# ZooMEISTER/vickers-hardness-Unet

Measured on AMD Instinct MI355X. Metric: 512x512 images/sec (train fwd+bwd), higher is better.
Workload: dtype bf16

## Files before the change

### vickers-hardness-unet_amd/csrc/conv_bwd_onepass.hip

```cpp
#include <stdlib.h>

#include <string>
#include <type_traits>

#include "vk_common.h"

namespace vk {

void launch_slab_reduce(size_t n4, int splits, const float* slab, float* dw, hipStream_t st);

struct OnePassParams {
  const void *g, *z, *z1, *w;
  void* y;
  const float *coef, *scale, *shift, *bnr_scale, *bnr_shift;
  double* sums;
  float* slab;
  int N, H, W, RS, RSsum, relu;
  uint32_t w_bytes, t_bytes;
};

template <int CK>
struct OnePassCfg {
  static constexpr int NSTEP = CK == 16 ? 5 : 9;
  static constexpr int APS = CK == 16 ? 48 : 96;
  static constexpr int VPP = CK / 8;
  static constexpr int NVEC = 18 * VPP;
  static constexpr int NLD = (NVEC + 63) / 64;
  static constexpr int ROWB = CK == 16 ? 1024 : 2048;
  static constexpr int V_OFF = 4 * ROWB, ZERO_OFF = 8 * ROWB;
  static constexpr int WAVE_LDS = 8 * ROWB + 64;
  static constexpr int RED = CK * 9 * CK * 4;
  static constexpr int SMEM = 4 * WAVE_LDS > RED ? 4 * WAVE_LDS : RED;
  static_assert(18 * APS <= ROWB && NLD <= 2, "row image");
};

template <typename T, int CK>
__global__ __launch_bounds__(256, (CK == 16 ? 2 : 1)) void conv_bwd_onepass_kernel(const OnePassParams p) {
  using Cfg = OnePassCfg<CK>;
  constexpr int NSTEP = Cfg::NSTEP, APS = Cfg::APS, VPP = Cfg::VPP, NVEC = Cfg::NVEC, NLD = Cfg::NLD, ROWB = Cfg::ROWB;
  constexpr int VE = 8, TC = CK / 16;
  static_assert(sizeof(T) == 2, "16-bit element types");
  extern __shared__ __attribute__((aligned(16))) char smem[];
  typedef __attribute__((address_space(3))) s16x4_t* lds_s16x4_ptr;
  const int RS = p.RS;
  const int tid = threadIdx.x, lane = tid & 63;
  const int wave = __builtin_amdgcn_readfirstlane(tid >> 6);
  char* const ring = smem + wave * Cfg::WAVE_LDS;
  char* const vring = ring + Cfg::V_OFF;
  const int strips_x = (p.W + 15) / 16, strips_y = (p.H + RS - 1) / RS;
  int sid = (int)blockIdx.x * 4 + wave;
  const bool active = sid < p.N * strips_y * strips_x;
  const int strip = sid;
  const int sx = sid % strips_x;
  sid /= strips_x;
  const int sy = sid % strips_y;
  const int n = sid / strips_y;
  const int x0 = sx * 16, ys = sy * RS, ye = min(p.H, ys + RS);
  const int li = lane & 15, kg = lane >> 4;

  f32x4_t wacc[9][TC][TC];
#pragma unroll
  for (int t = 0; t < 9; ++t)
#pragma unroll
    for (int a = 0; a < TC; ++a)
#pragma unroll
      for (int b = 0; b < TC; ++b) wacc[t][a][b] = f32x4_t{0.f, 0.f, 0.f, 0.f};

  if (active) {
    const __amdgpu_buffer_rsrc_t rsg = make_rsrc(p.g, p.t_bytes);
    const __amdgpu_buffer_rsrc_t rsz = make_rsrc(p.z, p.t_bytes);
    const __amdgpu_buffer_rsrc_t rs1 = make_rsrc(p.z1, p.t_bytes);
    const __amdgpu_buffer_rsrc_t rsw = make_rsrc(p.w, p.w_bytes);

    u32x4_t wf[NSTEP][TC];
#pragma unroll
    for (int st = 0; st < NSTEP; ++st)
#pragma unroll
      for (int a = 0; a < TC; ++a) {
        const int row = a * 16 + li;
        uint32_t off;
        bool ok = true;
        if (CK == 16) {
          const int tap = 2 * st + (kg >> 1);
          ok = tap < 9;
          off = (uint32_t)(((row * 9 + (8 - tap)) * 16 + (kg & 1) * VE) * 2);
        } else {
          const int pos = kg ^ (((row >> 2) & 1) << 1);
          off = (uint32_t)((((8 - st) * CK + row) * 4 + pos) * 16);
        }
        wf[st][a] = buf_load16(rsw, ok ? off : kOOB);
      }
    if (lane < 4) *reinterpret_cast<u32x4_t*>(ring + Cfg::ZERO_OFF + lane * 16) = u32x4_t{0, 0, 0, 0};

    int st_off[NLD], ld_col[NLD];
    bool xok[NLD];
#pragma unroll
    for (int q = 0; q < NLD; ++q) {
      const int v = lane + 64 * q;
      int hx = v / VPP, hv = v % VPP;
      if (VPP == 4) {
        if ((hx | 3) < 18) hx = (hx & ~3) | ((hx & 1) << 1) | ((hx >> 1) & 1);
      } else {
        if ((v | 15) < NVEC) { hx = (v & 7) | ((v >> 4) << 3); hv = (v >> 3) & 1; }
      }
      const int xs = x0 - 1 + hx;
      xok[q] = v < NVEC && (unsigned)xs < (unsigned)p.W;
      ld_col[q] = xs * CK + hv * VE;
      st_off[q] = v < NVEC ? hx * APS + hv * 16 : -1;
    }
    static_assert(VPP == 4 || NLD == 1, "C = 16: one staged vector per lane");
    const int hvl = VPP == 4 ? lane % VPP : (((lane | 15) < NVEC) ? (lane >> 3) & 1 : lane % VPP);
    const bool aff = p.scale != nullptr, relu = p.relu != 0;
    float sc[VE], sh[VE], ca[VE], cb[VE], cc[VE];
#pragma unroll
    for (int j = 0; j < VE; ++j) {
      sc[j] = aff ? p.scale[hvl * VE + j] : 1.f;
      sh[j] = aff ? p.shift[hvl * VE + j] : 0.f;
      ca[j] = p.coef[hvl * VE + j];
      cb[j] = p.coef[CK + hvl * VE + j];
      cc[j] = p.coef[2 * CK + hvl * VE + j];
    }
    struct RowQ {
      u32x4_t g[NLD], z[NLD], v[NLD];
    };
    auto issue = [&](int j, RowQ& r) {
      const bool rok = (unsigned)j < (unsigned)p.H;
#pragma unroll
      for (int q = 0; q < NLD; ++q) {
        const uint32_t off = (rok && xok[q]) ? (uint32_t)(((n * p.H + j) * p.W) * CK + ld_col[q]) * 2u : kOOB;
        r.g[q] = buf_load16(rsg, off);
        r.z[q] = buf_load16(rsz, off);
        r.v[q] = buf_load16(rs1, off);
      }
    };
    auto write_row = [&](int j, const RowQ& r) {
      const bool rok = (unsigned)j < (unsigned)p.H;
      const int slot = (j & 3) * ROWB;
#pragma unroll
      for (int q = 0; q < NLD; ++q) {
        if (st_off[q] < 0) continue;
        float gf[VE], zf[VE], o[VE];
        Vec16<T>::unpack(r.g[q], gf);
        Vec16<T>::unpack(r.z[q], zf);
#pragma unroll
        for (int e = 0; e < VE; ++e) o[e] = fmaf(ca[e], gf[e], fmaf(cb[e], zf[e], cc[e]));
        u32x4_t dz = Vec16<T>::pack(o);
        u32x4_t v = r.v[q];
        if (aff) v = AffineRelu<T>::run(v, sc, sh, relu);
        if (!(rok && xok[q])) {
          dz = u32x4_t{0, 0, 0, 0};
          v = u32x4_t{0, 0, 0, 0};
        }
        *reinterpret_cast<u32x4_t*>(ring + slot + st_off[q]) = dz;
        *reinterpret_cast<u32x4_t*>(vring + slot + st_off[q]) = v;
      }
    };

    int fr_r16[CK == 16 ? NSTEP : 1], fr_off16[CK == 16 ? NSTEP : 1];
    if (CK == 16) {
#pragma unroll
      for (int st = 0; st < NSTEP; ++st) {
        const int tap = 2 * st + (kg >> 1);
        const int r = tap / 3, sxx = tap - r * 3;
        fr_r16[st] = tap < 9 ? r : -100;
        fr_off16[st] = (li + sxx) * APS + (kg & 1) * 16;
      }
    }
    const int fr_base32 = kg * 16;
    const int lane_t = (4 * kg + (li >> 2)) * APS + (4 * (lane & 3)) * 2;
    auto tr = [](const char* q) { return __builtin_bit_cast(u32x2_t, __builtin_amdgcn_ds_read_tr16_b64_v4i16((lds_s16x4_ptr)(q))); };

// ... 50 lines not shown
    write_row(ys, pre[0]);
    auto row = [&](int y, auto ph_c) {
      constexpr int PH = decltype(ph_c)::value;
      write_row(y + 1, pre[(PH + 1) & 3]);
      issue(y + 4, pre[PH & 3]);
      z_issue(y + 1, zq[(PH & 1) ^ 1]);
      f32x4_t acc[TC];
#pragma unroll
      for (int a = 0; a < TC; ++a) acc[a] = f32x4_t{0.f, 0.f, 0.f, 0.f};
#pragma unroll
      for (int st = 0; st < NSTEP; ++st) {
        int addr;
        if (CK == 16) {
          const int vrow = y - 1 + fr_r16[st];
          addr = fr_r16[st] < 0 ? Cfg::ZERO_OFF : (vrow & 3) * ROWB + fr_off16[st];
        } else {
          const int r = st / 3, sxx = st - r * 3;
          addr = ((y - 1 + r) & 3) * ROWB + (li + sxx) * APS + fr_base32;
        }
        const u32x4_t xf = *reinterpret_cast<const u32x4_t*>(ring + addr);
#pragma unroll
        for (int a = 0; a < TC; ++a) acc[a] = Mma<T>::run(wf[st][a], xf, acc[a]);
      }
      __builtin_amdgcn_sched_barrier(0);
      const bool y_ok = y < p.H;
#pragma unroll
      for (int a = 0; a < TC; ++a) {
        float f[4] = {acc[a][0], acc[a][1], acc[a][2], acc[a][3]};
        (void)round_t(f);
        finish(a, f, y_ok ? out_off(a, y) : kOOB, x_ok && y_ok, zq[PH & 1][a]);
      }
      if constexpr ((PH & 1) == 1) {
        constexpr int SL = (PH + 3) & 3, SH = PH & 3;
        u32x4_t zf[TC];
#pragma unroll
        for (int a = 0; a < TC; ++a) {
          const u32x2_t lo = tr(ring + SL * ROWB + APS + lane_t + a * 32), hi = tr(ring + SH * ROWB + APS + lane_t + a * 32);
          zf[a] = u32x4_t{lo[0], lo[1], hi[0], hi[1]};
        }
#pragma unroll
        for (int r = 0; r < 3; ++r) {
          const int slo = ((PH + 2 + r) & 3) * ROWB, shi = ((PH + 3 + r) & 3) * ROWB;
#pragma unroll
          for (int s_ = 0; s_ < 3; ++s_) {
            u32x4_t vf[TC];
#pragma unroll
            for (int b = 0; b < TC; ++b) {
              const u32x2_t lo = tr(vring + slo + s_ * APS + lane_t + b * 32), hi = tr(vring + shi + s_ * APS + lane_t + b * 32);
              vf[b] = u32x4_t{lo[0], lo[1], hi[0], hi[1]};
            }
#pragma unroll
            for (int a = 0; a < TC; ++a)
#pragma unroll
              for (int b = 0; b < TC; ++b) wacc[r * 3 + s_][a][b] = Mma<T>::run(zf[a], vf[b], wacc[r * 3 + s_][a][b]);
          }
        }
      }
    };
    double* const sp = p.sums + (size_t)(strip % VK_STATS_REPLICAS) * 2 * CK;
    auto flush_sums = [&]() {
#pragma unroll
      for (int a = 0; a < TC; ++a)
#pragma unroll
        for (int e = 0; e < 4; ++e) {
          const float u = row16_sum(s1[a][e]), v = row16_sum(s2[a][e]);
          const int ch = a * 16 + kg * 4 + e;
          if (li == 0) {
            atomicAdd(sp + ch, (double)u);
            atomicAdd(sp + CK + ch, (double)v);
          }
          s1[a][e] = 0.f; s2[a][e] = 0.f;
        }
    };
    const int RSsum = p.RSsum;
    for (int yb = ys, left = RSsum; yb < ye; yb += 4) {
      row(yb, std::integral_constant<int, 0>{});
      row(yb + 1, std::integral_constant<int, 1>{});
      row(yb + 2, std::integral_constant<int, 2>{});
      row(yb + 3, std::integral_constant<int, 3>{});
      left -= 4;
      if (left == 0 || yb + 4 >= ye) {
        flush_sums();
        left = RSsum;
      }
    }
  }

  __syncthreads();
  float* const red = reinterpret_cast<float*>(smem);
#pragma unroll 1
  for (int phase = 0; phase < 4; ++phase) {
    if (wave == phase) {
#pragma unroll
      for (int t = 0; t < 9; ++t)
#pragma unroll
        for (int a = 0; a < TC; ++a)
#pragma unroll
          for (int b = 0; b < TC; ++b)
#pragma unroll
            for (int e = 0; e < 4; ++e) {
              const int k = a * 16 + kg * 4 + e, c = b * 16 + li;
              float* dst = red + (k * 9 + t) * CK + c;
              if (phase > 0) *dst += wacc[t][a][b][e];
              else *dst = wacc[t][a][b][e];
            }
    }
    __syncthreads();
  }
  float* const slab = p.slab + (size_t)blockIdx.x * CK * 9 * CK;
  for (int i = tid; i < CK * 9 * CK / 4; i += 256) *reinterpret_cast<f32x4_t*>(slab + i * 4) = *reinterpret_cast<const f32x4_t*>(red + i * 4);
}

template <typename T, int CK>
static int launch_onepass(OnePassParams p, float* dw, size_t slab_bytes, hipStream_t st) {
  using Cfg = OnePassCfg<CK>;
  const char* e_rs = getenv("VK_STREAM_RS");
  int RS = 256;
  if (e_rs) {
    RS = atoi(e_rs);
  } else {
    const long per_row_block = (long)p.N * ((p.W + 15) / 16), resident = CK == 16 ? 2048 : 1024;
    while (RS > 32 && per_row_block * ((p.H + RS - 1) / RS) < resident) RS >>= 1;
  }
  RS = (RS + 7) & ~7;
  if (RS < 8) RS = 8;
  int RSsum = RS;
  if (!e_rs) {
    const long per_row_block = (long)p.N * ((p.W + 15) / 16);
    RSsum = 32;
    while (RSsum * 2 <= 256 && per_row_block * ((p.H + 2 * RSsum - 1) / (2 * RSsum)) >= 4096) RSsum *= 2;
    if (RS < RSsum) RS = RSsum;
  }
  p.RSsum = RSsum;
  p.RS = RS;
  const long strips = (long)p.N * ((p.H + RS - 1) / RS) * ((p.W + 15) / 16);
  const long nwg = (strips + 3) / 4;
  if ((size_t)nwg * CK * 9 * CK * sizeof(float) > slab_bytes) return VK_ERR_UNSUPPORTED;
  static bool attr_done = false;
  if (!attr_done && Cfg::SMEM > 64 * 1024) {
    VK_CHECK_HIP(hipFuncSetAttribute((const void*)conv_bwd_onepass_kernel<T, CK>, hipFuncAttributeMaxDynamicSharedMemorySize, Cfg::SMEM));
    attr_done = true;
  }
  {
    static const std::string tag = std::string("bwd_onepass_16b_c") + std::to_string(CK);
    const double px = (double)p.N * p.H * p.W;
    vkh::ProfScope ps(tag.c_str(), st, 2.0 * 2.0 * px * CK * 9.0 * CK, 4.0 * px * CK * 2.0 + 9.0 * CK * CK * (2.0 + 4.0));
    hipLaunchKernelGGL((conv_bwd_onepass_kernel<T, CK>), dim3((unsigned)nwg), dim3(256), Cfg::SMEM, st, p);
  }
  launch_slab_reduce((size_t)CK * 9 * CK / 4, (int)nwg, p.slab, dw, st);
  VK_CHECK_HIP(hipGetLastError());
  return VK_OK;
}

}

extern "C" int vk_conv_bwd_onepass(const vk_conv_desc* d, const void* g, const void* z, const float* coef_abc, const void* w_dgrad, void* y,
                                   const vk_bnr* bnr, float* dw, void* workspace, size_t workspace_bytes, void* stream) {
  VK_CHECK_ARG(d && g && z && coef_abc && w_dgrad && y && bnr && dw, "vk_conv_bwd_onepass: null argument");
  if (d->dtype != VK_BF16 && d->dtype != VK_F16) return VK_ERR_UNSUPPORTED;
  if (d->R != 3 || d->S != 3 || d->stride != 1 || d->pad != 1 || d->transposed || d->H != d->Ho || d->W != d->Wo) return VK_ERR_UNSUPPORTED;
  if (d->src1.ptr || d->src0.up || d->src0.C != d->K || (d->K != 16 && d->K != 32)) return VK_ERR_UNSUPPORTED;
  if ((size_t)d->N * d->H * d->W * d->K * 2 >= (1ull << 31)) return VK_ERR_UNSUPPORTED;
  if (!workspace || (reinterpret_cast<uintptr_t>(workspace) & 15)) return VK_ERR_UNSUPPORTED;
  VK_CHECK_ARG(d->src0.ptr && d->N > 0 && d->H > 0 && d->W > 0, "vk_conv_bwd_onepass: empty descriptor");
  VK_CHECK_ARG((d->src0.scale != nullptr) == (d->src0.shift != nullptr), "vk_conv_bwd_onepass: scale and shift come together");
  VK_CHECK_ARG(bnr->z == d->src0.ptr && !bnr->mask && !bnr->accumulate && bnr->sums && bnr->scale && bnr->shift,
               "vk_conv_bwd_onepass: bnr must describe the layer's own input (z = src0.ptr, scale, shift, sums; no mask, no accumulate)");
  vk::OnePassParams p;
  p.g = g; p.z = z; p.z1 = d->src0.ptr; p.w = w_dgrad; p.y = y;
  p.coef = coef_abc; p.scale = d->src0.scale; p.shift = d->src0.shift; p.relu = d->src0.relu;
  p.bnr_scale = bnr->scale; p.bnr_shift = bnr->shift; p.sums = bnr->sums;
  p.slab = (float*)workspace;
  p.N = d->N; p.H = d->H; p.W = d->W; p.RS = 0;
  p.w_bytes = (uint32_t)((size_t)d->K * 9 * d->K * 2);
  p.t_bytes = (uint32_t)((size_t)d->N * d->H * d->W * d->K * 2);
  hipStream_t st = (hipStream_t)stream;
  if (d->dtype == VK_BF16)
    return d->K == 16 ? vk::launch_onepass<vk::bf16_t, 16>(p, dw, workspace_bytes, st) : vk::launch_onepass<vk::bf16_t, 32>(p, dw, workspace_bytes, st);
  return d->K == 16 ? vk::launch_onepass<vk::f16_t, 16>(p, dw, workspace_bytes, st) : vk::launch_onepass<vk::f16_t, 32>(p, dw, workspace_bytes, st);
}
```

### vickers-hardness-unet_amd/csrc/engine.hip

```cpp
#include <stdarg.h>
#include <stdio.h>
#include <stdlib.h>
#include <string.h>

#include <algorithm>
#include <atomic>
#include <map>
#include <mutex>
#include <string>
#include <vector>

#include "vk_common.h"

namespace vkh {
static thread_local char g_err[512] = "";
void set_error(const char* fmt, ...) {
  va_list ap;
  va_start(ap, fmt);
  vsnprintf(g_err, sizeof(g_err), fmt, ap);
  va_end(ap);
}

struct ProfRec {
  std::string tag;
// ... 1164 lines not shown
    xd = bn_act(h, c2);
  }
  vk_src hs = to_src(xd);
  if (h->classes == 1) RET_IF(vk_head_fwd(dt, N, S, SW, &hs, h->params + h->head_w_off, h->params + h->head_b_off, logits, st));
  else RET_IF(vk_head_fwd_multi(dt, N, S, SW, h->classes, &hs, h->params + h->head_w_off, h->params + h->head_b_off, logits, st));
  if (training) {
    if (h->bn_frozen_fwd) hipLaunchKernelGGL(k_inc_i64_masked, dim3(1), dim3(64), 0, st, (int)h->bns.size(), h->nbt, h->bn_frozen_fwd);
    else hipLaunchKernelGGL(k_inc_i64, dim3(1), dim3(64), 0, st, (int)h->bns.size(), h->nbt);
    VK_CHECK_HIP(hipGetLastError());
  }
  return VK_OK;
}

extern "C" int vk_unet_loss_ex(vk_unet* h, int mode, const void* logits, const void* target, float* loss_out, float grad_scale,
                               float w_ce, float w_dice, void* stream) {
  VK_CHECK_ARG(h && h->bound && logits && target && loss_out, "vk_unet_loss_ex: plan not bound or null tensor");
  VK_CHECK_ARG(mode == VK_LOSS_BINARY || mode == VK_LOSS_MULTILABEL || mode == VK_LOSS_MULTICLASS, "vk_unet_loss_ex: bad mode %d", mode);
  VK_CHECK_ARG(mode != VK_LOSS_BINARY || h->classes == 1, "vk_unet_loss_ex: the binary loss needs classes == 1 (the plan has %d)", h->classes);
  VK_CHECK_ARG(mode != VK_LOSS_MULTICLASS || h->classes >= 2, "vk_unet_loss_ex: the multi-class loss needs classes >= 2");
  if (h->classes == 1) return vk_unet_loss(h, (const float*)logits, (const float*)target, loss_out, grad_scale, w_ce, w_dice, stream);
  const int N = h->cfg.N, HW = h->cfg.size * h->cfg.width;
  float* dl = h->cfg.training ? (float*)(h->ws + h->off_dlogits) : nullptr;
  if (mode == VK_LOSS_MULTILABEL)
    return vk_multilabel_loss(N, h->classes, HW, (const float*)logits, (const float*)target, h->ws + h->off_mloss, h->mloss_bytes, loss_out,
                              dl, grad_scale, w_ce, w_dice, stream);
  return vk_multiclass_loss(N, h->classes, HW, (const float*)logits, (const int64_t*)target, h->ws + h->off_mloss, h->mloss_bytes, loss_out,
                            dl, grad_scale, w_ce, w_dice, stream);
}

extern "C" int vk_unet_loss_cfg(vk_unet* h, const vk_seg_loss_cfg* cfg, const void* logits, const void* target, float* loss_out,
                                float grad_scale, void* stream) {
  VK_CHECK_ARG(h && h->bound && cfg && logits && target && loss_out, "vk_unet_loss_cfg: plan not bound or null argument");
  float* dl = h->cfg.training ? (float*)(h->ws + h->off_dlogits) : nullptr;
  return vk_seg_loss(cfg, h->cfg.N, h->classes, h->cfg.size * h->cfg.width, (const float*)logits, target, h->ws + h->off_sloss,
                     h->sloss_bytes, loss_out, dl, grad_scale, stream);
}

extern "C" int vk_unet_loss_lovasz(vk_unet* h, const vk_seg_loss_cfg* seg_cfg, const vk_lovasz_cfg* lovasz_cfg, float w_lovasz,
                                   const void* logits, const void* target, void* workspace, size_t workspace_bytes, float* loss_out,
                                   float grad_scale, void* stream) {
  VK_CHECK_ARG(h && h->bound && lovasz_cfg && logits && target && workspace && loss_out,
               "vk_unet_loss_lovasz: plan not bound or null argument");
  VK_CHECK_ARG(w_lovasz == w_lovasz && w_lovasz - w_lovasz == 0.f, "vk_unet_loss_lovasz: w_lovasz is not finite");
  VK_CHECK_ARG(!seg_cfg || seg_cfg->mode == lovasz_cfg->mode, "vk_unet_loss_lovasz: the two parts disagree on the mode");
  const int N = h->cfg.N, HW = h->cfg.size * h->cfg.width;
  float* dl = h->cfg.training ? (float*)(h->ws + h->off_dlogits) : nullptr;
  hipStream_t st = (hipStream_t)stream;
  if (seg_cfg) RET_IF(vk_seg_loss(seg_cfg, N, h->classes, HW, (const float*)logits, target, h->ws + h->off_sloss, h->sloss_bytes, loss_out,
                                  dl, grad_scale, stream));
  else VK_CHECK_HIP(hipMemsetAsync(loss_out, 0, 8 * sizeof(float), st));
  RET_IF(vk_lovasz_loss(lovasz_cfg, N, h->classes, HW, (const float*)logits, target, workspace, workspace_bytes, loss_out + 8, dl,
                        grad_scale * w_lovasz, seg_cfg ? 1 : 0, stream));
  return vk::lovasz_combine(loss_out, w_lovasz, st);
}

extern "C" int vk_unet_loss(vk_unet* h, const float* logits, const float* target, float* loss_out, float grad_scale, float w_bce,
                            float w_dice, void* stream) {
  VK_CHECK_ARG(h && h->bound && logits && target && loss_out, "vk_unet_loss: plan not bound or null tensor");
  VK_CHECK_ARG(h->classes == 1, "vk_unet_loss: the binary loss needs classes == 1; use vk_unet_loss_ex");
  const size_t count = (size_t)h->cfg.N * h->cfg.size * h->cfg.width;
  float* dl = h->cfg.training ? (float*)(h->ws + h->off_dlogits) : nullptr;
  return vk_bce_dice_loss(count, logits, target, (double*)(h->ws + h->off_loss_sums), loss_out, dl, grad_scale, w_bce, w_dice, stream);
}

#ifndef VK_BN_APPLY_FUSED_MAXC_DEFAULT
#define VK_BN_APPLY_FUSED_MAXC_DEFAULT 0
#endif
namespace {

int bn_bwd_phase2(vk_unet* h, BnL& b, int C, size_t pixels, const void* dy, const void* z, int mask_mode, const void* mask_src, void* dz,
                  void* g_out, int g_acc, hipStream_t st) {
  static const int maxc = getenv("VK_BN_APPLY_FUSED_MAXC") ? atoi(getenv("VK_BN_APPLY_FUSED_MAXC")) : VK_BN_APPLY_FUSED_MAXC_DEFAULT;
  if (frozen(h, b)) {
    if (trains(h, b.g_t) || trains(h, b.b_t))
      RET_IF(vk_bn_bwd_coeffs_frozen(C, b.bsums, h->params + b.g_off, b.mean, b.invstd, dgamma_of(h, b), dbeta_of(h, b), b.coef, st));
    return vk_bn_bwd_apply(h->cfg.dtype, pixels, C, dy, z, mask_mode, b.scale, b.shift, mask_src, b.coef, dz, g_out, g_acc, st);
  }
  if (C <= maxc)
    return vk_bn_bwd_apply_fused(h->cfg.dtype, pixels, C, dy, z, mask_mode, b.scale, b.shift, mask_src, b.bsums, b.count, h->params + b.g_off,
                                 b.mean, b.invstd, dgamma_of(h, b), dbeta_of(h, b), dz, g_out, g_acc, st);
  RET_IF(vk_bn_bwd_coeffs(C, b.bsums, b.count, h->params + b.g_off, b.mean, b.invstd, dgamma_of(h, b), dbeta_of(h, b), b.coef, st));
  return vk_bn_bwd_apply(h->cfg.dtype, pixels, C, dy, z, mask_mode, b.scale, b.shift, mask_src, b.coef, dz, g_out, g_acc, st);
}

int bn_relu_bwd_inplace(vk_unet* h, ConvL& c, bool prereduced, hipStream_t st) {
  BnL& b = h->bns[c.bn];
  const size_t pixels = (size_t)h->cfg.N * c.Hout * c.Wout;
  if (!prereduced && bn_sums_needed(h, b)) RET_IF(vk_bn_bwd_reduce(h->cfg.dtype, pixels, c.K, c.g, c.z, 1, b.scale, b.shift, nullptr, b.bsums, st));
  return bn_bwd_phase2(h, b, c.K, pixels, c.g, c.z, prereduced ? 0 : 1, nullptr, c.g, nullptr, 0, st);
}

int wgrad_stream(vk_unet* h, hipStream_t st, hipStream_t* out) {
  *out = st;
  if (!h->side) return VK_OK;
  VK_CHECK_HIP(hipEventRecord(h->ev_fork, st));
  VK_CHECK_HIP(hipStreamWaitEvent(h->side, h->ev_fork, 0));
  h->side_dirty = true;
  *out = h->side;
  return VK_OK;
}

int join_side(vk_unet* h, hipStream_t st) {
  if (!h->side || !h->side_dirty) return VK_OK;
  VK_CHECK_HIP(hipEventRecord(h->ev_join, h->side));
  VK_CHECK_HIP(hipStreamWaitEvent(st, h->ev_join, 0));
  h->side_dirty = false;
  return VK_OK;
}

int conv_wgrad(vk_unet* h, ConvL& c, const vk_src& s0, const vk_src& s1, hipStream_t st) {
  vk_conv_desc d = conv_desc(h, c, s0, s1);
  if (!h->side && vk::wgrad_batch_supports(&d)) {
    h->pending.push_back(vk_unet::WItem{d, c.g, h->grads + c.w_off});
    return VK_OK;
  }
  hipStream_t ws;
  RET_IF(wgrad_stream(h, st, &ws));
  return vk_conv_wgrad(&d, c.g, h->grads + c.w_off, h->ws + h->off_wslab, VK_WGRAD_WORKSPACE_BYTES, ws);
}

vk_bnr bnr_of(vk_unet* h, ConvL& target) {
  BnL& b = h->bns[target.bn];
  vk_bnr r;
  r.z = target.z; r.scale = b.scale; r.shift = b.shift; r.sums = b.bsums; r.mask = nullptr; r.accumulate = 0;
  return r;
}

vk_conv_desc dgrad_desc(vk_unet* h, ConvL& c) {
  vk_conv_desc d;
  d.dtype = h->cfg.dtype;
  d.N = h->cfg.N; d.H = c.Hout; d.W = c.Wout; d.Ho = c.Hin; d.Wo = c.Win;
  d.K = c.Cin; d.R = c.R; d.S = c.R; d.stride = c.stride; d.pad = c.pad; d.transposed = 1;
  vk_src s;
  s.ptr = c.g; s.C = c.K; s.up = 0; s.scale = nullptr; s.shift = nullptr; s.relu = 0;
  d.src0 = s;
  d.src1 = null_src();
  return d;
}

int conv_dgrad_into(vk_unet* h, ConvL& c, ConvL& into, bool* fused, hipStream_t st) {
  vk_conv_desc d = dgrad_desc(h, c);
  if (on_1x1(c)) {
    *fused = false;
    return vk_conv1x1_fwd(&d, dgrad_weights(h, c), into.g, 0, nullptr, st);
  }
  vk_bnr r = bnr_of(h, into);
  int rc = getenv("VK_NO_BNR_FUSION") ? VK_ERR_UNSUPPORTED : vk_conv_dgrad_fused(&d, dgrad_weights(h, c), into.g, nullptr, 0, 0, &r, st);
  *fused = rc == VK_OK;
  if (rc != VK_ERR_UNSUPPORTED) return rc;
  if (c.halo_dg) return vk_conv_fwd_packed(&d, dgrad_weights(h, c), into.g, nullptr, 0, 0, nullptr, st);
  return vk_conv_fwd(&d, dgrad_weights(h, c), into.g, nullptr, 0, 0, nullptr, st);
}

int conv_bwd_onepass(vk_unet* h, ConvL& c, ConvL& into, int* state, hipStream_t st) {
  *state = 0;
  BnL& b = h->bns[c.bn];
  vk_conv_desc d = conv_desc(h, c, to_src(bn_act(h, into)), null_src());
  if (d.dtype == VK_F32 || d.R != 3 || d.S != 3 || d.stride != 1 || d.pad != 1 || d.src0.up || d.src0.C != d.K || (d.K != 16 && d.K != 32)) return VK_OK;
  static const int maxc = getenv("VK_BN_APPLY_FUSED_MAXC") ? atoi(getenv("VK_BN_APPLY_FUSED_MAXC")) : VK_BN_APPLY_FUSED_MAXC_DEFAULT;
  if (!frozen(h, b) && c.K <= maxc) return VK_OK;
  if (frozen(h, b)) {
    if (trains(h, b.g_t) || trains(h, b.b_t))
      RET_IF(vk_bn_bwd_coeffs_frozen(c.K, b.bsums, h->params + b.g_off, b.mean, b.invstd, dgamma_of(h, b), dbeta_of(h, b), b.coef, st));
  } else {
    RET_IF(vk_bn_bwd_coeffs(c.K, b.bsums, b.count, h->params + b.g_off, b.mean, b.invstd, dgamma_of(h, b), dbeta_of(h, b), b.coef, st));
  }
  vk_bnr r = bnr_of(h, into);
  const int rc = vk_conv_bwd_onepass(&d, c.g, c.z, b.coef, dgrad_weights(h, c), into.g, &r, h->grads + c.w_off, h->ws + h->off_wslab,
                                     VK_WGRAD_WORKSPACE_BYTES, st);
  if (rc == VK_ERR_UNSUPPORTED) {
    *state = 2;
    return vk_bn_bwd_apply(h->cfg.dtype, (size_t)h->cfg.N * c.Hout * c.Wout, c.K, c.g, c.z, 0, b.scale, b.shift, nullptr, b.coef, c.g, nullptr, 0, st);
  }
  *state = rc == VK_OK ? 1 : 0;
  return rc;
}

int conv_dgrad(vk_unet* h, ConvL& c, void* y, void* y1, int split, int accumulate, hipStream_t st) {
  vk_conv_desc d;
  d.dtype = h->cfg.dtype;
  d.N = h->cfg.N; d.H = c.Hout; d.W = c.Wout; d.Ho = c.Hin; d.Wo = c.Win;
  d.K = c.Cin; d.R = c.R; d.S = c.R; d.stride = c.stride; d.pad = c.pad; d.transposed = 1;
  vk_src s;
  s.ptr = c.g; s.C = c.K; s.up = 0; s.scale = nullptr; s.shift = nullptr; s.relu = 0;
  d.src0 = s;
  d.src1 = null_src();
  if (on_1x1(c) && !split) return vk_conv1x1_fwd(&d, dgrad_weights(h, c), y, accumulate, nullptr, st);
  if (c.halo_dg) return vk_conv_fwd_packed(&d, dgrad_weights(h, c), y, y1, split, accumulate, nullptr, st);
  return vk_conv_fwd(&d, dgrad_weights(h, c), y, y1, split, accumulate, nullptr, st);
}

int backward_decoder(vk_unet* h, int i, hipStream_t st) {
  DecL& d = h->decs[i];
  ConvL& c1 = h->convs[d.conv1];
  ConvL& c2 = h->convs[d.conv2];
  const int N = h->cfg.N;
  ConvL& stem = h->convs[h->stem_conv];
  Act xprev, skip{nullptr, 0, nullptr, nullptr, 0};
  void* g_prev;
  if (i == 0) {
    BlockL& f5 = h->blocks[h->layer_last_block[3]];
    xprev = Act{f5.out, f5.C, nullptr, nullptr, 0};
    g_prev = f5.gout;
  } else {
    ConvL& pc2 = h->convs[h->decs[i - 1].conv2];
    xprev = bn_act(h, pc2);
    g_prev = pc2.g;
  }
  void* g_skip = nullptr;
  if (i <= 2) {
    BlockL& fb = h->blocks[h->layer_last_block[2 - i]];
    skip = Act{fb.out, fb.C, nullptr, nullptr, 0};
    g_skip = fb.gout;
  } else if (i == 3) {
    skip = bn_act(h, stem);
    g_skip = stem.g;
  }
  const BnL& bn1 = h->bns[c1.bn];
  if (!need_from(h, h->bns[c2.bn].rank)) {
    if (i > 0) h->g_prereduced[h->decs[i - 1].conv2] = 0;
    return VK_OK;
  }
  const bool into1 = need_from(h, bn1.rank);
  bool fused1 = false;
  int onepass = 0;
  if (h->g_prereduced[d.conv2] && into1 && trains(h, c2.w_t) && h->cfg.dtype != VK_F32 && !h->side && !on_1x1(c2) && !getenv("VK_NO_ONEPASS") &&
      !getenv("VK_NO_BNR_FUSION"))
    RET_IF(conv_bwd_onepass(h, c2, c1, &onepass, st));
  if (onepass == 1) {
    fused1 = true;
  } else {
    if (onepass == 0) RET_IF(bn_relu_bwd_inplace(h, c2, h->g_prereduced[d.conv2] != 0, st));
    if (into1) RET_IF(conv_dgrad_into(h, c2, c1, &fused1, st));
    if (trains(h, c2.w_t)) RET_IF(conv_wgrad(h, c2, to_src(bn_act(h, c1)), null_src(), st));
  }
  if (i > 0) h->g_prereduced[h->decs[i - 1].conv2] = 0;
  if (!into1) return VK_OK;
  RET_IF(bn_relu_bwd_inplace(h, c1, fused1, st));
  if (need_from(h, c1.rank + 1)) {
    vk_conv_desc dd = dgrad_desc(h, c1);
    vk_bnr r;
    const bool want_bnr = i > 0 && !getenv("VK_NO_BNR_FUSION");
    if (want_bnr) r = bnr_of(h, h->convs[h->decs[i - 1].conv2]);
    const int rc = vk_conv_dgrad_fused(&dd, dgrad_weights(h, c1), g_prev, d.Cskip ? g_skip : nullptr, d.Cskip ? d.Cup : 0, 1,
                                       want_bnr ? &r : nullptr, st);
    if (rc == VK_OK && want_bnr) h->g_prereduced[h->decs[i - 1].conv2] = 1;
    if (rc != VK_OK && rc != VK_ERR_UNSUPPORTED) return rc;
    if (rc == VK_ERR_UNSUPPORTED) {
      void* dup = h->ws + h->off_dup;
      if (d.Cskip) RET_IF(conv_dgrad(h, c1, dup, g_skip, d.Cup, 0, st));
      else RET_IF(conv_dgrad(h, c1, dup, nullptr, 0, 0, st));
      RET_IF(vk_upsample2x_bwd(h->cfg.dtype, N, d.H, d.W, d.Cup, dup, g_prev, 0, st));
    }
  }
  if (!trains(h, c1.w_t)) return VK_OK;
  return conv_wgrad(h, c1, to_src(xprev, 1), d.Cskip ? to_src(skip) : null_src(), st);
}

int backward_block(vk_unet* h, int bi, hipStream_t st) {
  BlockL& k = h->blocks[bi];
  ConvL& c1 = h->convs[k.conv1];
  ConvL& c2 = h->convs[k.conv2];
  BnL& b2 = h->bns[c2.bn];
  const vk_dtype dt = h->cfg.dtype;
  const size_t pixels = (size_t)h->cfg.N * k.Hout * k.Wout;
  if (!need_from(h, b2.rank)) {
    h->tail_prereduced[(size_t)bi] = 0;
    return VK_OK;
  }
  Act xin;
  void* gin;
  if (bi == 0) {
    xin = Act{h->ws + h->off_pool, 64, nullptr, nullptr, 0};
    gin = h->ws + h->off_gpool;
  } else {
    BlockL& pb = h->blocks[bi - 1];
    xin = Act{pb.out, pb.C, nullptr, nullptr, 0};
    gin = pb.gout;
  }
  const bool pre = h->tail_prereduced[(size_t)bi] != 0;
  h->tail_prereduced[(size_t)bi] = 0;
  if (bi > 0) h->tail_prereduced[(size_t)bi - 1] = 0;
  const int mm = pre ? 0 : 2;
  if (!pre && bn_sums_needed(h, b2)) RET_IF(vk_bn_bwd_reduce(dt, pixels, k.C, k.gout, c2.z, 2, nullptr, nullptr, k.out, b2.bsums, st));
  if (k.convd < 0) {
    RET_IF(bn_bwd_phase2(h, b2, k.C, pixels, k.gout, c2.z, mm, k.out, c2.g, gin, k.in_has_grad_first ? 1 : 0, st));
  } else {
    ConvL& cd = h->convs[k.convd];
    BnL& bd = h->bns[cd.bn];
    RET_IF(bn_bwd_phase2(h, b2, k.C, pixels, k.gout, c2.z, mm, k.out, c2.g, nullptr, 0, st));
    if (bn_sums_needed(h, bd)) RET_IF(vk_bn_bwd_reduce(dt, pixels, k.C, k.gout, cd.z, mm, nullptr, nullptr, k.out, bd.bsums, st));
    RET_IF(bn_bwd_phase2(h, bd, k.C, pixels, k.gout, cd.z, mm, k.out, cd.g, nullptr, 0, st));
  }
  const bool into1 = need_from(h, h->bns[c1.bn].rank);
  bool fused1 = false;
  if (into1) RET_IF(conv_dgrad_into(h, c2, c1, &fused1, st));
  if (trains(h, c2.w_t)) RET_IF(conv_wgrad(h, c2, to_src(bn_act(h, c1)), null_src(), st));
  if (!into1) return k.convd >= 0 && trains(h, h->convs[k.convd].w_t) ? conv_wgrad(h, h->convs[k.convd], to_src(xin), null_src(), st) : VK_OK;
  RET_IF(bn_relu_bwd_inplace(h, c1, fused1, st));
  const bool into_gin = need_from(h, c1.rank + 1);
  bool tail_fused = false;
  const int tail_maxc = getenv("VK_TAIL_BNR_MAXC") ? atoi(getenv("VK_TAIL_BNR_MAXC")) : 1 << 20;
  if (into_gin && k.convd < 0 && bi > 0 && c1.halo_dg && k.C <= tail_maxc && !getenv("VK_NO_TAIL_BNR_FUSION")) {
    BlockL& pb = h->blocks[bi - 1];
    ConvL& pc2 = h->convs[pb.conv2];
    vk_conv_desc dd = dgrad_desc(h, c1);
    vk_bnr r;
    r.z = pc2.z; r.scale = nullptr; r.shift = nullptr; r.sums = h->bns[pc2.bn].bsums; r.mask = pb.out; r.accumulate = 1;
    const int rc = vk_conv_dgrad_fused(&dd, dgrad_weights(h, c1), gin, nullptr, 0, 0, &r, st);
    if (rc == VK_OK) { tail_fused = true; h->tail_prereduced[(size_t)bi - 1] = 1; }
    else if (rc != VK_ERR_UNSUPPORTED) return rc;
  }
  if (into_gin && !tail_fused) RET_IF(conv_dgrad(h, c1, gin, nullptr, 0, 1, st));
  if (k.convd >= 0) {
    ConvL& cd = h->convs[k.convd];
    if (into_gin) RET_IF(conv_dgrad(h, cd, gin, nullptr, 0, 1, st));
    if (trains(h, c1.w_t)) RET_IF(conv_wgrad(h, c1, to_src(xin), null_src(), st));
    return trains(h, cd.w_t) ? conv_wgrad(h, cd, to_src(xin), null_src(), st) : VK_OK;
  }
  return trains(h, c1.w_t) ? conv_wgrad(h, c1, to_src(xin), null_src(), st) : VK_OK;
}

int backward_bottleneck(vk_unet* h, int bi, hipStream_t st) {
  BlockL& k = h->blocks[bi];
  ConvL& c1 = h->convs[k.conv1];
  ConvL& c2 = h->convs[k.conv2];
  ConvL& c3 = h->convs[k.conv3];
  BnL& b3 = h->bns[c3.bn];
  const vk_dtype dt = h->cfg.dtype;
  const size_t pixels = (size_t)h->cfg.N * k.Hout * k.Wout;
  h->tail_prereduced[(size_t)bi] = 0;
  if (!need_from(h, b3.rank)) return VK_OK;
  Act xin;
  void* gin;
  if (bi == 0) {
    xin = Act{h->ws + h->off_pool, 64, nullptr, nullptr, 0};
    gin = h->ws + h->off_gpool;
  } else {
    BlockL& pb = h->blocks[bi - 1];
    xin = Act{pb.out, pb.C, nullptr, nullptr, 0};
    gin = pb.gout;
  }
  bool gin_written = k.in_has_grad_first;
  if (bn_sums_needed(h, b3)) RET_IF(vk_bn_bwd_reduce(dt, pixels, k.C, k.gout, c3.z, 2, nullptr, nullptr, k.out, b3.bsums, st));
  if (k.convd < 0) {
    RET_IF(bn_bwd_phase2(h, b3, k.C, pixels, k.gout, c3.z, 2, k.out, c3.g, gin, gin_written ? 1 : 0, st));
    gin_written = true;
  } else {
    RET_IF(bn_bwd_phase2(h, b3, k.C, pixels, k.gout, c3.z, 2, k.out, c3.g, nullptr, 0, st));
    ConvL& cd = h->convs[k.convd];
    BnL& bd = h->bns[cd.bn];
    if (need_from(h, bd.rank)) {
      if (bn_sums_needed(h, bd)) RET_IF(vk_bn_bwd_reduce(dt, pixels, k.C, k.gout, cd.z, 2, nullptr, nullptr, k.out, bd.bsums, st));
      RET_IF(bn_bwd_phase2(h, bd, k.C, pixels, k.gout, cd.z, 2, k.out, cd.g, nullptr, 0, st));
    }
  }
  const bool into2 = need_from(h, h->bns[c2.bn].rank);
  if (into2) RET_IF(conv_dgrad(h, c3, c2.g, nullptr, 0, 0, st));
  if (trains(h, c3.w_t)) RET_IF(conv_wgrad(h, c3, to_src(bn_act(h, c2)), null_src(), st));
  if (k.convd >= 0 && trains(h, h->convs[k.convd].w_t)) RET_IF(conv_wgrad(h, h->convs[k.convd], to_src(xin), null_src(), st));
  if (!into2) return VK_OK;
  RET_IF(bn_relu_bwd_inplace(h, c2, false, st));
  const bool into1 = need_from(h, h->bns[c1.bn].rank);
  bool fused1 = false;
  if (into1) RET_IF(conv_dgrad_into(h, c2, c1, &fused1, st));
  if (trains(h, c2.w_t)) RET_IF(conv_wgrad(h, c2, to_src(bn_act(h, c1)), null_src(), st));
  if (!into1) return VK_OK;
  RET_IF(bn_relu_bwd_inplace(h, c1, fused1, st));
  if (need_from(h, c1.rank + 1)) {
    RET_IF(conv_dgrad(h, c1, gin, nullptr, 0, gin_written ? 1 : 0, st));
    if (k.convd >= 0) RET_IF(conv_dgrad(h, h->convs[k.convd], gin, nullptr, 0, 1, st));
  }
  return trains(h, c1.w_t) ? conv_wgrad(h, c1, to_src(xin), null_src(), st) : VK_OK;
}

int stem_coeffs(vk_unet* h, BnL& b, hipStream_t st) {
  if (!frozen(h, b))
    return vk_bn_bwd_coeffs(64, b.bsums, b.count, h->params + b.g_off, b.mean, b.invstd, dgamma_of(h, b), dbeta_of(h, b), b.coef, st);
  if (!trains(h, b.g_t) && !trains(h, b.b_t)) return VK_OK;
  return vk_bn_bwd_coeffs_frozen(64, b.bsums, h->params + b.g_off, b.mean, b.invstd, dgamma_of(h, b), dbeta_of(h, b), b.coef, st);
}

int backward_stem(vk_unet* h, hipStream_t st) {
  const int N = h->cfg.N, S = h->cfg.size, SW = h->cfg.width;
  ConvL& stem = h->convs[h->stem_conv];
  if (!need_from(h, h->bns[stem.bn].rank)) return VK_OK;
  BnL& b = h->bns[stem.bn];
  const bool want_w = trains(h, stem.w_t);
  const float* const w = h->params + stem.w_off;
  if (getenv("VK_NO_POOL_BNR_FUSION")) {
    RET_IF(vk_maxpool_bwd(h->cfg.dtype, N, S / 2, SW / 2, 64, h->ws + h->off_gpool, (const uint8_t*)(h->ws + h->off_argmax), stem.g, st));
// ... 124 lines not shown
```

Baseline: 3060.

## Add fused one-pass backward kernel for upsampled decoder conv without skip

```diff
diff --git a/vickers-hardness-unet_amd/csrc/conv_bwd_onepass.hip b/vickers-hardness-unet_amd/csrc/conv_bwd_onepass.hip
--- a/vickers-hardness-unet_amd/csrc/conv_bwd_onepass.hip
+++ b/vickers-hardness-unet_amd/csrc/conv_bwd_onepass.hip
@@ -16,7 +16,7 @@
   double* sums;
   float* slab;
   int N, H, W, RS, RSsum, relu;
-  uint32_t w_bytes, t_bytes;
+  uint32_t w_bytes, t_bytes, t1_bytes;
 };
 
 template <int CK>
@@ -373,6 +373,360 @@
   return VK_OK;
 }
 
+struct OnePassUpCfg {
+  static constexpr int NSTEP = 5, APS = 48, ROWB = 1024;
+  static constexpr int VSB = 96, VROW = 18 * VSB;
+  static constexpr int V_OFF = 4 * ROWB, ZERO_OFF = V_OFF + 4 * VROW;
+  static constexpr int TAB_OFF = ZERO_OFF + 64, TAB_SC = 48, TAB_SH = 80, TAB_BSC = 112, TAB_BSH = 144, TAB_N = 176;
+  static constexpr int WAVE_LDS = TAB_OFF + TAB_N * 4;
+  static constexpr int K = 16, C = 32;
+  static constexpr int RED = K * 9 * C * 4;
+  static constexpr int SMEM = 4 * WAVE_LDS > RED ? 4 * WAVE_LDS : RED;
+  static_assert(18 * APS <= ROWB && WAVE_LDS % 16 == 0, "row images");
+};
+
+template <typename T>
+__global__ __launch_bounds__(256, 2) void conv_bwd_onepass_up_kernel(const OnePassParams p) {
+  using Cfg = OnePassUpCfg;
+  constexpr int NSTEP = Cfg::NSTEP, APS = Cfg::APS, ROWB = Cfg::ROWB, VSB = Cfg::VSB, VROW = Cfg::VROW;
+  constexpr int VE = 8, TC = 2, K = Cfg::K, C = Cfg::C;
+  static_assert(sizeof(T) == 2, "16-bit element types");
+  extern __shared__ __attribute__((aligned(16))) char smem[];
+  typedef __attribute__((address_space(3))) s16x4_t* lds_s16x4_ptr;
+  const int RS = p.RS;
+  const int tid = threadIdx.x, lane = tid & 63;
+  const int wave = __builtin_amdgcn_readfirstlane(tid >> 6);
+  char* const ring = smem + wave * Cfg::WAVE_LDS;
+  char* const vring = ring + Cfg::V_OFF;
+  const int strips_x = (p.W + 15) / 16, strips_y = (p.H + RS - 1) / RS;
+  int sid = (int)blockIdx.x * 4 + wave;
+  const bool active = sid < p.N * strips_y * strips_x;
+  const int strip = sid;
+  const int sx = sid % strips_x;
+  sid /= strips_x;
+  const int sy = sid % strips_y;
+  const int n = sid / strips_y;
+  const int x0 = sx * 16, ys = sy * RS, ye = min(p.H, ys + RS);
+  const int li = lane & 15, kg = lane >> 4;
+  const int Hs = p.H >> 1, Ws = p.W >> 1;
+
+  f32x4_t wacc[9][TC];
+#pragma unroll
+  for (int t = 0; t < 9; ++t)
+#pragma unroll
+    for (int b = 0; b < TC; ++b) wacc[t][b] = f32x4_t{0.f, 0.f, 0.f, 0.f};
+
+  if (active) {
+    const __amdgpu_buffer_rsrc_t rsg = make_rsrc(p.g, p.t_bytes);
+    const __amdgpu_buffer_rsrc_t rsz = make_rsrc(p.z, p.t_bytes);
+    const __amdgpu_buffer_rsrc_t rs1 = make_rsrc(p.z1, p.t1_bytes);
+    const __amdgpu_buffer_rsrc_t rsw = make_rsrc(p.w, p.w_bytes);
+
+    u32x4_t wf[NSTEP][TC];
+#pragma unroll
+    for (int st = 0; st < NSTEP; ++st)
+#pragma unroll
+      for (int a = 0; a < TC; ++a) {
+        const int tap = 2 * st + (kg >> 1);
+        const uint32_t off = (uint32_t)((((a * 16 + li) * 9 + (8 - tap)) * 16 + (kg & 1) * VE) * 2);
+        wf[st][a] = buf_load16(rsw, tap < 9 ? off : kOOB);
+      }
+    if (lane < 4) *reinterpret_cast<u32x4_t*>(ring + Cfg::ZERO_OFF + lane * 16) = u32x4_t{0, 0, 0, 0};
+
+    int d_off, d_col;
+    bool d_xok;
+    int hvd;
+    {
+      int hx = lane >> 1;
+      hvd = lane & 1;
+      if ((lane | 15) < 36) { hx = (lane & 7) | ((lane >> 4) << 3); hvd = (lane >> 3) & 1; }
+      const int xs = x0 - 1 + hx;
+      d_xok = lane < 36 && (unsigned)xs < (unsigned)p.W;
+      d_col = xs * K + hvd * VE;
+      d_off = lane < 36 ? hx * APS + hvd * 16 : -1;
+    }
+    const int vj = lane >> 2;
+    const int vcs = (x0 >> 1) - 1 + vj;
+    const bool v_lane = lane < 40, v_xok = v_lane && (unsigned)vcs < (unsigned)Ws;
+    const int v_col = vcs * C + (lane & 3) * VE;
+    const bool aff = p.scale != nullptr, relu = p.relu != 0;
+    float* const tab = reinterpret_cast<float*>(ring + Cfg::TAB_OFF);
+    for (int i = lane; i < Cfg::TAB_N; i += 64) {
+      float v;
+      if (i < Cfg::TAB_SC) v = p.coef[i];
+      else if (i < Cfg::TAB_SH) v = aff ? p.scale[i - Cfg::TAB_SC] : 1.f;
+      else if (i < Cfg::TAB_BSC) v = aff ? p.shift[i - Cfg::TAB_SH] : 0.f;
+      else if (i < Cfg::TAB_BSH) v = p.bnr_scale[i - Cfg::TAB_BSC];
+      else v = p.bnr_shift[i - Cfg::TAB_BSH];
+      tab[i] = v;
+    }
+    const float* const tab_d = tab + hvd * VE;
+    const float* const tab_v = tab + (lane & 3) * VE;
+    const float* const tab_o = tab + kg * 4;
+    auto ld8 = [](const float* q, float (&o)[VE]) {
+      const f32x4_t lo = *reinterpret_cast<const f32x4_t*>(q), hi = *reinterpret_cast<const f32x4_t*>(q + 4);
+#pragma unroll
+      for (int e = 0; e < 4; ++e) { o[e] = lo[e]; o[4 + e] = hi[e]; }
+    };
+    struct RowQ {
+      u32x4_t g, z;
+    };
+    auto issue = [&](int j, RowQ& r) {
+      const bool ok = (unsigned)j < (unsigned)p.H && d_xok;
+      const uint32_t off = ok ? (uint32_t)(((n * p.H + j) * p.W) * K + d_col) * 2u : kOOB;
+      r.g = buf_load16(rsg, off);
+      r.z = buf_load16(rsz, off);
+    };
+    auto issue_v = [&](int m, u32x4_t& r) {
+      const bool ok = (unsigned)m < (unsigned)Hs && v_xok;
+      r = buf_load16(rs1, ok ? (uint32_t)(((n * Hs + m) * Ws) * C + v_col) * 2u : kOOB);
+    };
+    auto write_row = [&](int j, const RowQ& r) {
+      if (d_off < 0) return;
+      float gf[VE], zf[VE], o[VE], ca[VE], cb[VE], cc[VE];
+      ld8(tab_d, ca);
+      ld8(tab_d + K, cb);
+      ld8(tab_d + 2 * K, cc);
+      Vec16<T>::unpack(r.g, gf);
+      Vec16<T>::unpack(r.z, zf);
+#pragma unroll
+      for (int e = 0; e < VE; ++e) o[e] = fmaf(ca[e], gf[e], fmaf(cb[e], zf[e], cc[e]));
+      u32x4_t dz = Vec16<T>::pack(o);
+      if (!((unsigned)j < (unsigned)p.H && d_xok)) dz = u32x4_t{0, 0, 0, 0};
+      *reinterpret_cast<u32x4_t*>(ring + (j & 3) * ROWB + d_off) = dz;
+    };
+    auto write_v = [&](int m, const u32x4_t& r) {
+      if (!v_lane) return;
+      u32x4_t x = r;
+      if (aff) {
+        float sc[VE], sh[VE];
+        ld8(tab_v + Cfg::TAB_SC, sc);
+        ld8(tab_v + Cfg::TAB_SH, sh);
+        x = AffineRelu<T>::run(x, sc, sh, relu);
+      }
+      if (!((unsigned)m < (unsigned)Hs && v_xok)) x = u32x4_t{0, 0, 0, 0};
+      char* const dst = vring + (m & 3) * VROW + (lane & 3) * 16;
+      if (vj > 0) *reinterpret_cast<u32x4_t*>(dst + (2 * vj - 1) * VSB) = x;
+      if (vj < 9) *reinterpret_cast<u32x4_t*>(dst + (2 * vj) * VSB) = x;
+    };
+
+    int fr_r16[NSTEP], fr_off16[NSTEP];
+#pragma unroll
+    for (int st = 0; st < NSTEP; ++st) {
+      const int tap = 2 * st + (kg >> 1);
+      const int r = tap / 3, sxx = tap - r * 3;
+      fr_r16[st] = tap < 9 ? r : -100;
+      fr_off16[st] = (li + sxx) * APS + (kg & 1) * 16;
+    }
+    const int lane_z = (4 * kg + (li >> 2) + 1) * APS + (4 * (lane & 3)) * 2;
+    const int lane_v = (4 * kg + (li >> 2)) * VSB + (4 * (lane & 3)) * 2;
+    auto tr = [](const char* q) { return __builtin_bit_cast(u32x2_t, __builtin_amdgcn_ds_read_tr16_b64_v4i16((lds_s16x4_ptr)(q))); };
+
+    const int xo = x0 + li;
+    const bool lane_stores = xo < p.W && (li & 1) == 0;
+    float s1[TC][4], s2[TC][4], prev[TC][4];
+#pragma unroll
+    for (int a = 0; a < TC; ++a)
+#pragma unroll
+      for (int e = 0; e < 4; ++e) {
+        s1[a][e] = 0.f; s2[a][e] = 0.f; prev[a][e] = 0.f;
+      }
+    auto round_t = [&](float (&f)[4]) {
+      float g[8] = {f[0], f[1], f[2], f[3], 0.f, 0.f, 0.f, 0.f};
+      const u32x4_t pk = Vec16<T>::pack(g);
+      Vec16<T>::unpack(pk, g);
+#pragma unroll
+      for (int e = 0; e < 4; ++e) f[e] = g[e];
+      return u32x2_t{pk[0], pk[1]};
+    };
+    const uint32_t lane_ob = lane_stores ? (uint32_t)(((n * Hs) * Ws + (xo >> 1)) * C + kg * 4) * 2u : kOOB;
+    const uint32_t row_ob = (uint32_t)(Ws * C * 2);
+    auto out_off = [&](int a, int y) -> uint32_t { return lane_ob + (uint32_t)(y >> 1) * row_ob + (uint32_t)(a * 32); };
+    u32x2_t zq[2][TC];
+    auto z_issue = [&](int y, u32x2_t (&z)[TC]) {
+      const bool ok = y < p.H;
+#pragma unroll
+      for (int a = 0; a < TC; ++a) z[a] = __builtin_amdgcn_raw_buffer_load_b64(rs1, ok ? out_off(a, y) : kOOB, 0, 0);
+    };
+    auto finish = [&](int a, float (&f)[4], uint32_t boff, bool counted, u32x2_t zr) {
+      float zf[8];
+      Vec16<T>::unpack(u32x4_t{zr[0], zr[1], 0u, 0u}, zf);
+      const f32x4_t bsc = *reinterpret_cast<const f32x4_t*>(tab_o + Cfg::TAB_BSC + a * 16);
+      const f32x4_t bsh = *reinterpret_cast<const f32x4_t*>(tab_o + Cfg::TAB_BSH + a * 16);
+#pragma unroll
+      for (int e = 0; e < 4; ++e) {
+        if (!counted || !(fmaf(zf[e], bsc[e], bsh[e]) > 0.f)) f[e] = 0.f;
+        s1[a][e] += f[e];
+        s2[a][e] += f[e] * zf[e];
+      }
+      const u32x2_t pk = round_t(f);
+      if ((int32_t)boff >= 0) *reinterpret_cast<u32x2_t*>((char*)p.y + boff) = pk;
+    };
+
+    RowQ pre[4];
+    u32x4_t vq[2], v0, v1;
+    const int ss = ys >> 1;
+    issue(ys - 1, pre[3]);
+    issue(ys, pre[0]);
+    issue_v(ss - 1, v0);
+    issue_v(ss, v1);
+    issue(ys + 1, pre[1]);
+    issue(ys + 2, pre[2]);
+    issue_v(ss + 1, vq[1]);
+    issue_v(ss + 2, vq[0]);
+    z_issue(ys + 1, zq[0]);
+    write_row(ys - 1, pre[3]);
+    issue(ys + 3, pre[3]);
+    write_row(ys, pre[0]);
+    write_v(ss - 1, v0);
+    write_v(ss, v1);
+    auto row = [&](int y, auto ph_c) {
+      constexpr int PH = decltype(ph_c)::value;
+      write_row(y + 1, pre[(PH + 1) & 3]);
+      issue(y + 4, pre[PH & 3]);
+      constexpr int ZC = (PH >> 1) & 1;
+      if constexpr ((PH & 1) == 1) {
+        constexpr int VS = ((PH + 1) >> 1) & 1;
+        const int m1 = (y + 1) >> 1;
+        write_v(m1, vq[VS]);
+        issue_v(m1 + 2, vq[VS]);
+        z_issue(y + 2, zq[ZC ^ 1]);
+      }
+      f32x4_t acc[TC];
+#pragma unroll
+      for (int a = 0; a < TC; ++a) acc[a] = f32x4_t{0.f, 0.f, 0.f, 0.f};
+#pragma unroll
+      for (int st = 0; st < NSTEP; ++st) {
+        const int vrow = y - 1 + fr_r16[st];
+        const int addr = fr_r16[st] < 0 ? Cfg::ZERO_OFF : (vrow & 3) * ROWB + fr_off16[st];
+        const u32x4_t xf = *reinterpret_cast<const u32x4_t*>(ring + addr);
+#pragma unroll
+        for (int a = 0; a < TC; ++a) acc[a] = Mma<T>::run(wf[st][a], xf, acc[a]);
+      }
+      __builtin_amdgcn_sched_barrier(0);
+      const bool y_ok = y < p.H;
+#pragma unroll
+      for (int a = 0; a < TC; ++a) {
+        float f[4] = {acc[a][0], acc[a][1], acc[a][2], acc[a][3]};
+        (void)round_t(f);
+        if constexpr ((PH & 1) == 0) {
+#pragma unroll
+          for (int e = 0; e < 4; ++e) prev[a][e] = f[e];
+        } else {
+          float t[4];
+#pragma unroll
+          for (int e = 0; e < 4; ++e) {
+            const float pn = dpp_f<0xB1>(prev[a][e]), cn = dpp_f<0xB1>(f[e]);
+            t[e] = ((prev[a][e] + pn) + f[e]) + cn;
+          }
+          (void)round_t(t);
+          finish(a, t, y_ok ? out_off(a, y) : kOOB, lane_stores && y_ok, zq[ZC][a]);
+        }
+      }
+      if constexpr ((PH & 1) == 1) {
+        constexpr int SL = (PH + 3) & 3, SH = PH & 3;
+        const u32x2_t zlo = tr(ring + SL * ROWB + lane_z), zhi = tr(ring + SH * ROWB + lane_z);
+        const u32x4_t zf = u32x4_t{zlo[0], zlo[1], zhi[0], zhi[1]};
+        const int m = y >> 1;
+        const char* const Va = vring + ((m - 1) & 3) * VROW + lane_v;
+        const char* const Vb = vring + (m & 3) * VROW + lane_v;
+        const char* const Vc = vring + ((m + 1) & 3) * VROW + lane_v;
+#pragma unroll
+        for (int s_ = 0; s_ < 3; ++s_)
+#pragma unroll
+          for (int b = 0; b < TC; ++b) {
+            const u32x2_t va = tr(Va + s_ * VSB + b * 32), vb = tr(Vb + s_ * VSB + b * 32), vc = tr(Vc + s_ * VSB + b * 32);
+            wacc[s_][b] = Mma<T>::run(zf, u32x4_t{va[0], va[1], vb[0], vb[1]}, wacc[s_][b]);
+            wacc[3 + s_][b] = Mma<T>::run(zf, u32x4_t{vb[0], vb[1], vb[0], vb[1]}, wacc[3 + s_][b]);
+            wacc[6 + s_][b] = Mma<T>::run(zf, u32x4_t{vb[0], vb[1], vc[0], vc[1]}, wacc[6 + s_][b]);
+          }
+      }
+    };
+    double* const sp = p.sums + (size_t)(strip % VK_STATS_REPLICAS) * 2 * C;
+    auto flush_sums = [&]() {
+#pragma unroll
+      for (int a = 0; a < TC; ++a)
+#pragma unroll
+        for (int e = 0; e < 4; ++e) {
+          const float u = row16_sum(s1[a][e]), v = row16_sum(s2[a][e]);
+          const int ch = a * 16 + kg * 4 + e;
+          if (li == 0) {
+            atomicAdd(sp + ch, (double)u);
+            atomicAdd(sp + C + ch, (double)v);
+          }
+          s1[a][e] = 0.f; s2[a][e] = 0.f;
+        }
+    };
+    const int RSsum = p.RSsum;
+    for (int yb = ys, left = RSsum; yb < ye; yb += 4) {
+      row(yb, std::integral_constant<int, 0>{});
+      row(yb + 1, std::integral_constant<int, 1>{});
+      row(yb + 2, std::integral_constant<int, 2>{});
+      row(yb + 3, std::integral_constant<int, 3>{});
+      left -= 4;
+      if (left == 0 || yb + 4 >= ye) {
+        flush_sums();
+        left = RSsum;
+      }
+    }
+  }
+
+  __syncthreads();
+  float* const red = reinterpret_cast<float*>(smem);
+#pragma unroll 1
+  for (int phase = 0; phase < 4; ++phase) {
+    if (wave == phase) {
+#pragma unroll
+      for (int t = 0; t < 9; ++t)
+#pragma unroll
+        for (int b = 0; b < TC; ++b)
+#pragma unroll
+          for (int e = 0; e < 4; ++e) {
+            float* dst = red + ((kg * 4 + e) * 9 + t) * C + b * 16 + li;
+            if (phase > 0) *dst += wacc[t][b][e];
+            else *dst = wacc[t][b][e];
+          }
+    }
+    __syncthreads();
+  }
+  float* const slab = p.slab + (size_t)blockIdx.x * K * 9 * C;
+  for (int i = tid; i < K * 9 * C / 4; i += 256) *reinterpret_cast<f32x4_t*>(slab + i * 4) = *reinterpret_cast<const f32x4_t*>(red + i * 4);
+}
+
+template <typename T>
+static int launch_onepass_up(OnePassParams p, float* dw, size_t slab_bytes, hipStream_t st) {
+  using Cfg = OnePassUpCfg;
+  const char* e_rs = getenv("VK_STREAM_RS");
+  const long per_row_block = (long)p.N * ((p.W + 15) / 16);
+  int RS = 256;
+  if (e_rs) {
+    RS = atoi(e_rs);
+  } else {
+    while (RS > 32 && per_row_block * ((p.H + RS - 1) / RS) < 2048) RS >>= 1;
+  }
+  RS = (RS + 7) & ~7;
+  if (RS < 8) RS = 8;
+  int RSsum = RS;
+  if (!e_rs) {
+    RSsum = 32;
+    while (RSsum * 2 <= 256 && per_row_block * ((p.H + 2 * RSsum - 1) / (2 * RSsum)) >= 4096) RSsum *= 2;
+    if (RS < RSsum) RS = RSsum;
+  }
+  p.RSsum = RSsum;
+  p.RS = RS;
+  const long strips = (long)p.N * ((p.H + RS - 1) / RS) * ((p.W + 15) / 16);
+  const long nwg = (strips + 3) / 4;
+  if ((size_t)nwg * Cfg::K * 9 * Cfg::C * sizeof(float) > slab_bytes) return VK_ERR_UNSUPPORTED;
+  {
+    const double px = (double)p.N * p.H * p.W;
+    vkh::ProfScope ps("bwd_onepass_16b_c32up_k16", st, 2.0 * 2.0 * px * Cfg::K * 9.0 * Cfg::C, 3.0 * px * Cfg::K * 2.0 + 9.0 * Cfg::K * Cfg::C * (2.0 + 4.0));
+    hipLaunchKernelGGL((conv_bwd_onepass_up_kernel<T>), dim3((unsigned)nwg), dim3(256), Cfg::SMEM, st, p);
+  }
+  launch_slab_reduce((size_t)Cfg::K * 9 * Cfg::C / 4, (int)nwg, p.slab, dw, st);
+  VK_CHECK_HIP(hipGetLastError());
+  return VK_OK;
+}
+
 }
 
 extern "C" int vk_conv_bwd_onepass(const vk_conv_desc* d, const void* g, const void* z, const float* coef_abc, const void* w_dgrad, void* y,
@@ -380,7 +734,9 @@
   VK_CHECK_ARG(d && g && z && coef_abc && w_dgrad && y && bnr && dw, "vk_conv_bwd_onepass: null argument");
   if (d->dtype != VK_BF16 && d->dtype != VK_F16) return VK_ERR_UNSUPPORTED;
   if (d->R != 3 || d->S != 3 || d->stride != 1 || d->pad != 1 || d->transposed || d->H != d->Ho || d->W != d->Wo) return VK_ERR_UNSUPPORTED;
-  if (d->src1.ptr || d->src0.up || d->src0.C != d->K || (d->K != 16 && d->K != 32)) return VK_ERR_UNSUPPORTED;
+  const bool up = d->src0.up != 0;
+  if (d->src1.ptr) return VK_ERR_UNSUPPORTED;
+  if (up ? (d->src0.C != 32 || d->K != 16 || ((d->H | d->W) & 1)) : (d->src0.C != d->K || (d->K != 16 && d->K != 32))) return VK_ERR_UNSUPPORTED;
   if ((size_t)d->N * d->H * d->W * d->K * 2 >= (1ull << 31)) return VK_ERR_UNSUPPORTED;
   if (!workspace || (reinterpret_cast<uintptr_t>(workspace) & 15)) return VK_ERR_UNSUPPORTED;
   VK_CHECK_ARG(d->src0.ptr && d->N > 0 && d->H > 0 && d->W > 0, "vk_conv_bwd_onepass: empty descriptor");
@@ -393,9 +749,11 @@
   p.bnr_scale = bnr->scale; p.bnr_shift = bnr->shift; p.sums = bnr->sums;
   p.slab = (float*)workspace;
   p.N = d->N; p.H = d->H; p.W = d->W; p.RS = 0;
-  p.w_bytes = (uint32_t)((size_t)d->K * 9 * d->K * 2);
   p.t_bytes = (uint32_t)((size_t)d->N * d->H * d->W * d->K * 2);
+  p.t1_bytes = up ? (uint32_t)((size_t)d->N * (d->H / 2) * (d->W / 2) * d->src0.C * 2) : p.t_bytes;
+  p.w_bytes = (uint32_t)((size_t)d->K * 9 * d->src0.C * 2);
   hipStream_t st = (hipStream_t)stream;
+  if (up) return d->dtype == VK_BF16 ? vk::launch_onepass_up<vk::bf16_t>(p, dw, workspace_bytes, st) : vk::launch_onepass_up<vk::f16_t>(p, dw, workspace_bytes, st);
   if (d->dtype == VK_BF16)
     return d->K == 16 ? vk::launch_onepass<vk::bf16_t, 16>(p, dw, workspace_bytes, st) : vk::launch_onepass<vk::bf16_t, 32>(p, dw, workspace_bytes, st);
   return d->K == 16 ? vk::launch_onepass<vk::f16_t, 16>(p, dw, workspace_bytes, st) : vk::launch_onepass<vk::f16_t, 32>(p, dw, workspace_bytes, st);
diff --git a/vickers-hardness-unet_amd/csrc/engine.hip b/vickers-hardness-unet_amd/csrc/engine.hip
--- a/vickers-hardness-unet_amd/csrc/engine.hip
+++ b/vickers-hardness-unet_amd/csrc/engine.hip
@@ -1340,11 +1340,12 @@
   return vk_conv_fwd(&d, dgrad_weights(h, c), into.g, nullptr, 0, 0, nullptr, st);
 }
 
-int conv_bwd_onepass(vk_unet* h, ConvL& c, ConvL& into, int* state, hipStream_t st) {
+int conv_bwd_onepass(vk_unet* h, ConvL& c, ConvL& into, int up, int* state, hipStream_t st) {
   *state = 0;
   BnL& b = h->bns[c.bn];
-  vk_conv_desc d = conv_desc(h, c, to_src(bn_act(h, into)), null_src());
-  if (d.dtype == VK_F32 || d.R != 3 || d.S != 3 || d.stride != 1 || d.pad != 1 || d.src0.up || d.src0.C != d.K || (d.K != 16 && d.K != 32)) return VK_OK;
+  vk_conv_desc d = conv_desc(h, c, to_src(bn_act(h, into), up), null_src());
+  if (d.dtype == VK_F32 || d.R != 3 || d.S != 3 || d.stride != 1 || d.pad != 1) return VK_OK;
+  if (up ? (d.src0.C != 32 || d.K != 16 || ((d.H | d.W) & 1)) : (d.src0.C != d.K || (d.K != 16 && d.K != 32))) return VK_OK;
   static const int maxc = getenv("VK_BN_APPLY_FUSED_MAXC") ? atoi(getenv("VK_BN_APPLY_FUSED_MAXC")) : VK_BN_APPLY_FUSED_MAXC_DEFAULT;
   if (!frozen(h, b) && c.K <= maxc) return VK_OK;
   if (frozen(h, b)) {
@@ -1414,7 +1415,7 @@
   int onepass = 0;
   if (h->g_prereduced[d.conv2] && into1 && trains(h, c2.w_t) && h->cfg.dtype != VK_F32 && !h->side && !on_1x1(c2) && !getenv("VK_NO_ONEPASS") &&
       !getenv("VK_NO_BNR_FUSION"))
-    RET_IF(conv_bwd_onepass(h, c2, c1, &onepass, st));
+    RET_IF(conv_bwd_onepass(h, c2, c1, 0, &onepass, st));
   if (onepass == 1) {
     fused1 = true;
   } else {
@@ -1424,7 +1425,15 @@
   }
   if (i > 0) h->g_prereduced[h->decs[i - 1].conv2] = 0;
   if (!into1) return VK_OK;
-  RET_IF(bn_relu_bwd_inplace(h, c1, fused1, st));
+  int onepass1 = 0;
+  if (fused1 && i > 0 && !d.Cskip && trains(h, c1.w_t) && need_from(h, c1.rank + 1) && h->cfg.dtype != VK_F32 && !h->side && !on_1x1(c1) &&
+      !getenv("VK_NO_ONEPASS") && !getenv("VK_NO_ONEPASS_UP") && !getenv("VK_NO_BNR_FUSION"))
+    RET_IF(conv_bwd_onepass(h, c1, h->convs[h->decs[i - 1].conv2], 1, &onepass1, st));
+  if (onepass1 == 1) {
+    h->g_prereduced[h->decs[i - 1].conv2] = 1;
+    return VK_OK;
+  }
+  if (onepass1 == 0) RET_IF(bn_relu_bwd_inplace(h, c1, fused1, st));
   if (need_from(h, c1.rank + 1)) {
     vk_conv_desc dd = dgrad_desc(h, c1);
     vk_bnr r;
```

Result: faster. 3094, median of 6 (+1.1%).
